# navi0105/LyricAlignment

Measured on AMD Instinct MI355X. Metric: aligned audio-sec/sec (RTF^-1), Whisper-medium 30 s clips, higher is better.
Workload: dtype bf16; 1 GPU; whisper-medium encoder + BiGRU/FC head + CTC forced alignment, batch 32 x 30 s mel per GPU (BASELINE.json configs[1]); clips_per_gpu=32, frames=1500, vocab=21129, labels_per_clip=5..26 (one per sung note), pipeline=2 encoder stream(s) + 1 head stream, head over 4 batches

## Files before the change

lyricalignment_amd/csrc/la_attention.hip:

```cpp
#include <type_traits>

#include "la_common.h"

using la::bf16_t;

namespace {

typedef __attribute__((ext_vector_type(16))) float f32x16;
typedef __attribute__((ext_vector_type(8))) __bf16 bf16x8;
typedef __attribute__((ext_vector_type(8))) _Float16 f16x8;

template <typename T16> struct Half16;
template <> struct Half16<bf16_t> {
    typedef bf16x8 vec8;
    typedef __bf16 elem;
    static constexpr unsigned kOnes = 0x3F803F80u;
    static constexpr float kPLimit = 0x1p30f;
    __device__ static __forceinline__ f32x16 mfma32(vec8 a, vec8 b, f32x16 c) { return __builtin_amdgcn_mfma_f32_32x32x16_bf16(a, b, c, 0, 0, 0); }
};
template <> struct Half16<la::f16_t> {
    typedef f16x8 vec8;
    typedef _Float16 elem;
    static constexpr unsigned kOnes = 0x3C003C00u;
    static constexpr float kPLimit = 0x1p13f;
    __device__ static __forceinline__ f32x16 mfma32(vec8 a, vec8 b, f32x16 c) { return __builtin_amdgcn_mfma_f32_32x32x16_f16(a, b, c, 0, 0, 0); }
};
typedef __attribute__((ext_vector_type(4))) short s16x4;

constexpr int QT = 128;
constexpr int KT = 64;
constexpr float kLog2e = 1.4426950408889634f;

struct AttnParams {
    const void *q, *k, *v;
    int64_t ld_q, ld_kv;
    void *out;
    int64_t ld_out;
    int q_len, kv_len, n_head, causal;
    int64_t q_bs, kv_bs, out_bs;
    int batch;
    float defer_thr;
    float *lse = nullptr;
    float score_scale = 1.4426950408889634f;
};

struct BlockCoord { int qt, head, clip; };
__device__ __forceinline__ BlockCoord block_coord(int nq, int n_head, int batch) {
    const int L = blockIdx.x, pairs = n_head * batch;
    int pair, qt;
    if ((pairs & 7) == 0) {
        const int x = L & 7, idx = L >> 3;
        pair = x + 8 * (idx / nq);
        qt = idx % nq;
    } else {
        pair = L / nq;
        qt = L % nq;
    }
    return BlockCoord{qt, pair % n_head, pair / n_head};
}

__device__ __forceinline__ int acc_row(int reg, int h) { return (reg & 3) + 8 * (reg >> 2) + 4 * h; }

__device__ __forceinline__ void glds16(const void *g, void *l) {
    la::glds16(g, l);
}

__device__ __forceinline__ int kswz(int r) { return (r >> 1) & 7; }
__device__ __forceinline__ int vswz(int r) { return ((r >> 1) & 1) << 2; }

struct KvOff { unsigned k[2], v[2]; };
template <int PER>
__device__ __forceinline__ KvOff kv_offsets_bf16(int64_t ld, int key0, int T, int wave, int lane) {
    KvOff o;
    const int r8 = lane >> 3, ps = lane & 7;
#pragma unroll
    for (int i = 0; i < PER; ++i) {
        const int r = (wave * PER + i) * 8 + r8;
        int rr = key0 + r < T ? r : T - 1 - key0;
        o.k[i] = (unsigned)(rr * ld * 2) + ((ps ^ kswz(r)) << 4);
        o.v[i] = (unsigned)(rr * ld * 2) + ((ps ^ vswz(r)) << 4);
    }
    return o;
}
template <int PER>
__device__ __forceinline__ void stage_kv_bf16(const bf16_t *kbase, const bf16_t *vbase, int64_t ld, int key0, const KvOff &o,
                                              unsigned kl, unsigned vl, int wave) {
    const bf16_t *ks = kbase + (int64_t)key0 * ld, *vs = vbase + (int64_t)key0 * ld;
#pragma unroll
    for (int i = 0; i < PER; ++i) {
        la::glds16_so(o.k[i], ks, kl + (wave * PER + i) * 1024);
        la::glds16_so(o.v[i], vs, vl + (wave * PER + i) * 1024);
    }
}

template <typename T16, int NW = 4, bool MSUM = false, int KO = 0, bool OPT = false, int PRIO = 0, bool FOLD = false>
__global__ __launch_bounds__(64 * NW, FOLD ? 4 : 2) void attention_bf16_kernel(AttnParams p) {
    static_assert(!(OPT && MSUM), "the optimistic form tests the vector-pipe row sums");
    static_assert(!FOLD || OPT, "the log2-domain form is a variant of the optimistic one");
    constexpr int QT = 32 * NW, PER = 8 / NW;
    typedef Half16<T16> HT;
    typedef typename HT::vec8 vec8;
    __shared__ __attribute__((aligned(16))) unsigned char lds[2 * 2 * KT * 128];
    const int T = p.kv_len;
    const BlockCoord bc = block_coord((p.q_len + QT - 1) / QT, p.n_head, p.batch);
    const int qt = bc.qt, head = bc.head, clip = bc.clip;
    const int tid = threadIdx.x, lane = tid & 63;
    const int wave = __builtin_amdgcn_readfirstlane(tid >> 6);
    const int i32 = lane & 31, h = lane >> 5;
    const bf16_t *base = reinterpret_cast<const bf16_t *>(p.q) + (int64_t)clip * p.q_bs * p.ld_q + head * 64;
    const bf16_t *kbase = reinterpret_cast<const bf16_t *>(p.k) + (int64_t)clip * p.kv_bs * p.ld_kv + head * 64;
    const bf16_t *vbase = reinterpret_cast<const bf16_t *>(p.v) + (int64_t)clip * p.kv_bs * p.ld_kv + head * 64;

    int qrow = qt * QT + wave * 32 + i32;
    const bool q_valid = qrow < p.q_len;
    qrow = q_valid ? qrow : p.q_len - 1;
    uint4 qf[4];
#pragma unroll
    for (int c = 0; c < 4; ++c) qf[c] = *reinterpret_cast<const uint4 *>(base + (int64_t)qrow * p.ld_q + 16 * c + 8 * h);

    f32x16 o[2];
#pragma unroll
    for (int b = 0; b < 2; ++b)
#pragma unroll
        for (int r = 0; r < 16; ++r) o[b][r] = 0.f;
    float m_run = FOLD ? 0.f : -INFINITY, l_part = 0.f;
    int plain = FOLD ? 1 : 0;
    const float kScale = FOLD ? 1.0f : p.score_scale;
    f32x16 osum;
#pragma unroll
    for (int r = 0; r < 16; ++r) osum[r] = 0.f;
    const uint4 ones4 = uint4{HT::kOnes, HT::kOnes, HT::kOnes, HT::kOnes};

    int nkv = (T + KT - 1) / KT;
    const int nkv_all = nkv;
    if (p.causal) nkv = min(nkv, (min(p.q_len, (qt + 1) * QT) - 1) / KT + 1);
    const unsigned lds0 = __builtin_amdgcn_readfirstlane(la::lds_addr_u32(lds));
    const KvOff off_full = kv_offsets_bf16<PER>(p.ld_kv, 0, KT, wave, lane);
    const KvOff off_last = kv_offsets_bf16<PER>(p.ld_kv, (nkv_all - 1) * KT, T, wave, lane);
    stage_kv_bf16<PER>(kbase, vbase, p.ld_kv, 0, nkv_all == 1 ? off_last : off_full, lds0, lds0 + KT * 128, wave);
    asm volatile("s_waitcnt vmcnt(0)" ::: "memory");
#pragma unroll
    for (int c = 0; c < 4; ++c) {
        typedef unsigned u32x4 __attribute__((ext_vector_type(4)));
        u32x4 t = __builtin_bit_cast(u32x4, qf[c]);
        asm volatile("" : "+v"(t));
        qf[c] = __builtin_bit_cast(uint4, t);
    }
    __syncthreads();

    const int g = lane >> 4, q4 = (lane & 15) >> 2, pp = lane & 3;

    auto tile = [&](int t, auto curc) __attribute__((always_inline)) {
        constexpr int cur = decltype(curc)::value;
        const unsigned char *kl = lds + cur * (2 * KT * 128);
        const unsigned char *vl = kl + KT * 128;
        if (t + 1 < nkv && !(KO & 8)) {
            const unsigned nk = lds0 + (cur ^ 1) * (2 * KT * 128);
            stage_kv_bf16<PER>(kbase, vbase, p.ld_kv, (t + 1) * KT, t + 2 == nkv_all ? off_last : off_full, nk, nk + KT * 128, wave);
        }
        f32x16 s[2];
        typedef std::integral_constant<int, 0> Sub0;
        typedef std::integral_constant<int, 1> Sub1;
        typedef std::integral_constant<int, 2> SubBoth;
        auto scores = [&](auto serialc, auto whichc) {
            constexpr bool serial = decltype(serialc)::value;
            constexpr int lo = decltype(whichc)::value == 2 ? 0 : decltype(whichc)::value;
            constexpr int hi = decltype(whichc)::value == 2 ? 2 : lo + 1;
            uint4 kf[2][4];
#pragma unroll
            for (int sub = lo; sub < hi; ++sub)
#pragma unroll
                for (int r = 0; r < 16; ++r) s[sub][r] = 0.f;
            if constexpr (!serial) {
#pragma unroll
                for (int c = 0; c < 4; ++c)
#pragma unroll
                    for (int sub = lo; sub < hi; ++sub) {
                        const int row = sub * 32 + i32;
                        if constexpr (KO & 4) kf[sub][c] = qf[(c + sub) & 3];
                        else kf[sub][c] = *reinterpret_cast<const uint4 *>(kl + row * 128 + (((2 * c + h) ^ kswz(row)) << 4));
                    }
            }
#pragma unroll
            for (int c = 0; c < 4; ++c) {
                if constexpr (serial) {
#pragma unroll
                    for (int sub = lo; sub < hi; ++sub) {
                        const int row = sub * 32 + i32;
                        kf[sub][c] = *reinterpret_cast<const uint4 *>(kl + row * 128 + (((2 * c + h) ^ kswz(row)) << 4));
                    }
                }
#pragma unroll
                for (int sub = lo; sub < hi; ++sub)
                    if constexpr (KO & 16) s[sub][c] += __builtin_bit_cast(float, kf[sub][c].x) + __builtin_bit_cast(float, kf[sub][c].w);
                    else s[sub] = HT::mfma32(__builtin_bit_cast(vec8, kf[sub][c]), __builtin_bit_cast(vec8, qf[c]), s[sub]);
                if constexpr (serial) __builtin_amdgcn_sched_barrier(0);
            }
            if ((t + 1) * KT > T || p.causal) {
                const int kmax = p.causal ? min(T - 1, qrow) : T - 1;
#pragma unroll
                for (int sub = lo; sub < hi; ++sub)
#pragma unroll
                    for (int r = 0; r < 16; ++r)
                        if (t * KT + sub * 32 + acc_row(r, h) > kmax) s[sub][r] = -INFINITY;
            }
        };
        typedef float f32x2 __attribute__((ext_vector_type(2)));
        auto exponentials = [&](float m, auto whichc) -> float {
            constexpr int lo = decltype(whichc)::value == 2 ? 0 : decltype(whichc)::value;
            constexpr int hi = decltype(whichc)::value == 2 ? 2 : lo + 1;
            float ps0 = 0.f, ps1 = 0.f;
            auto body = [&](auto subtract_m) {
#pragma unroll
                for (int sub = lo; sub < hi; ++sub)
#pragma unroll
                    for (int r = 0; r < 16; r += 2) {
                        float a0, a1;
                        if constexpr (FOLD) {
                            a0 = s[sub][r]; a1 = s[sub][r + 1];
                            if constexpr (decltype(subtract_m)::value) { a0 -= m; a1 -= m; }
                        } else { a0 = fmaf(s[sub][r], kScale, -m); a1 = fmaf(s[sub][r + 1], kScale, -m); }
                        const float p0 = (KO & 1) ? a0 : __builtin_amdgcn_exp2f(a0), p1 = (KO & 1) ? a1 : __builtin_amdgcn_exp2f(a1);
                        s[sub][r] = p0;
                        s[sub][r + 1] = p1;
                        if constexpr (!MSUM) { ps0 += p0; ps1 += p1; }
                    }
            };
            if (FOLD && plain) body(std::false_type{});
            else body(std::true_type{});
            return ps0 + ps1;
        };
        auto tile_max = [&](auto whichc) -> float {
            constexpr int lo = decltype(whichc)::value == 2 ? 0 : decltype(whichc)::value;
            constexpr int hi = decltype(whichc)::value == 2 ? 2 : lo + 1;
            float mx = -INFINITY;
#pragma unroll
            for (int sub = lo; sub < hi; ++sub)
#pragma unroll
                for (int r = 0; r < 16; ++r) mx = fmaxf(mx, s[sub][r]);
            return fmaxf(mx, __shfl_xor(mx, 32)) * kScale;
        };
        auto rescale = [&](float alpha) {
#pragma unroll
            for (int b = 0; b < 2; ++b)
#pragma unroll
                for (int r = 0; r < 16; ++r) o[b][r] *= alpha;
            if constexpr (MSUM) {
#pragma unroll
                for (int r = 0; r < 16; ++r) osum[r] *= alpha;
            }
        };
        auto pv_sub = [&](auto subc) {
            constexpr int sub = decltype(subc)::value;
#pragma unroll
            for (int ks = 0; ks < 2; ++ks) {
                vec8 pf;
#pragma unroll
                for (int j = 0; j < 8; ++j) pf[j] = (typename HT::elem)s[sub][8 * ks + j];
                if constexpr (MSUM) osum = HT::mfma32(__builtin_bit_cast(vec8, ones4), pf, osum);
#pragma unroll
                for (int b = 0; b < 2; ++b) {
                    const int key0 = sub * 32 + 16 * ks + 4 * (g >> 1);
                    const int slot = b * 4 + 2 * (g & 1) + (pp >> 1);
                    const int r0 = key0 + q4, r1 = key0 + 8 + q4;
                    typedef __attribute__((ext_vector_type(8))) short s16x8;
                    s16x8 vf;
                    if constexpr (KO & 2) vf = __builtin_bit_cast(s16x8, qf[(2 * sub + ks + b) & 3]);
                    else {
                        const s16x4 v0 = __builtin_amdgcn_ds_read_tr16_b64_v4i16(
                            (__attribute__((address_space(3))) s16x4 *)(vl + r0 * 128 + ((slot ^ vswz(r0)) << 4) + (pp & 1) * 8));
                        const s16x4 v1 = __builtin_amdgcn_ds_read_tr16_b64_v4i16(
                            (__attribute__((address_space(3))) s16x4 *)(vl + r1 * 128 + ((slot ^ vswz(r1)) << 4) + (pp & 1) * 8));
                        vf = __builtin_shufflevector(v0, v1, 0, 1, 2, 3, 4, 5, 6, 7);
                    }
                    if constexpr (KO & 16) o[b][2 * sub + ks] += (float)vf[0] + (float)vf[7] + (float)pf[0] + (float)pf[7];
                    else o[b] = HT::mfma32(__builtin_bit_cast(vec8, vf), pf, o[b]);
                }
            }
        };
        auto redo = [&](auto whichc) -> float {
            scores(std::true_type{}, whichc);
            const float m_new = fmaxf(m_run, tile_max(whichc));
            const float alpha = __builtin_amdgcn_exp2f(m_run - m_new);
            m_run = m_new;
            plain = 0;
            rescale(alpha);
            l_part *= alpha;
            return exponentials(m_new, whichc);
        };
        if constexpr (PRIO == 1 || PRIO == 2) __builtin_amdgcn_s_setprio(3);
        scores(std::false_type{}, SubBoth{});
        if constexpr (PRIO == 1 || PRIO == 2) __builtin_amdgcn_s_setprio(0);
        if constexpr (PRIO == 3) __builtin_amdgcn_s_setprio(3);
        if constexpr (OPT) {
            float ps0 = exponentials(m_run, Sub0{});
            if (__builtin_expect(__builtin_amdgcn_ballot_w64(!(ps0 <= HT::kPLimit)) != 0, 0)) ps0 = redo(Sub0{});
            l_part += ps0;
            float ps1 = exponentials(m_run, Sub1{});
            pv_sub(Sub0{});
            if (__builtin_expect(__builtin_amdgcn_ballot_w64(!(ps1 <= HT::kPLimit)) != 0, 0)) ps1 = redo(Sub1{});
            l_part += ps1;
            if constexpr (PRIO == 3) __builtin_amdgcn_s_setprio(0);
            if constexpr (PRIO == 2) __builtin_amdgcn_s_setprio(3);
            pv_sub(Sub1{});
            if constexpr (PRIO == 2) __builtin_amdgcn_s_setprio(0);
        } else {
            const float mx2 = tile_max(SubBoth{});
            float m_new = m_run, alpha = 1.0f;
            if (__builtin_amdgcn_ballot_w64(mx2 > m_run + p.defer_thr) != 0) {
                m_new = fmaxf(m_run, mx2);
                alpha = __builtin_amdgcn_exp2f(m_run - m_new);
            }
            m_run = m_new;
            const float ps = exponentials(m_new, SubBoth{});
            if constexpr (!MSUM) l_part = l_part * alpha + ps;
            if (__builtin_amdgcn_ballot_w64(alpha != 1.0f) != 0) rescale(alpha);
            pv_sub(Sub0{});
            pv_sub(Sub1{});
        }
        asm volatile("s_waitcnt vmcnt(0)" ::: "memory");
        if constexpr (!(KO & 32)) __syncthreads();
    };
    auto sweep = [&]() __attribute__((always_inline)) {
        for (int t = 0; t < nkv; t += 2) {
            tile(t, std::integral_constant<int, 0>{});
            if (t + 1 < nkv) tile(t + 1, std::integral_constant<int, 1>{});
        }
    };
    sweep();
    if constexpr (FOLD) {
        const float l0 = l_part + __shfl_xor(l_part, 32);
        if (__builtin_amdgcn_readfirstlane(__syncthreads_or(q_valid && !(l0 >= 0x1p-100f && l0 <= 0x1p100f)))) {
#pragma unroll
            for (int b = 0; b < 2; ++b)
#pragma unroll
                for (int r = 0; r < 16; ++r) o[b][r] = 0.f;
            m_run = -INFINITY; l_part = 0.f; plain = 0;
            stage_kv_bf16<PER>(kbase, vbase, p.ld_kv, 0, nkv_all == 1 ? off_last : off_full, lds0, lds0 + KT * 128, wave);
            asm volatile("s_waitcnt vmcnt(0)" ::: "memory");
            __syncthreads();
            sweep();
        }
    }

    const float l = MSUM ? osum[0] : l_part + __shfl_xor(l_part, 32);
    const float inv = 1.0f / l;
    if (q_valid) {
        bf16_t *orow = reinterpret_cast<bf16_t *>(p.out) + ((int64_t)clip * p.out_bs + qrow) * p.ld_out + head * 64;
#pragma unroll
        for (int b = 0; b < 2; ++b)
#pragma unroll
            for (int r4 = 0; r4 < 4; ++r4) {
                *reinterpret_cast<ushort4 *>(orow + 32 * b + 8 * r4 + 4 * h) =
                    la::Pack4<T16>::run(o[b][4 * r4 + 0] * inv, o[b][4 * r4 + 1] * inv, o[b][4 * r4 + 2] * inv, o[b][4 * r4 + 3] * inv);
            }
    }
}

__device__ __forceinline__ void stage_kv_f32(const float *kbase, const float *vbase, int64_t ld, int key0, int T,
                                             unsigned char *kl, unsigned char *vl, int wave, int lane) {
    const int r4 = lane >> 4, ps = lane & 15;
#pragma unroll
    for (int i = 0; i < 4; ++i) {
        const int piece = wave * 4 + i;
        const int r = piece * 4 + r4;
        int key = key0 + r;
        key = key < T ? key : T - 1;
        const int ls = ps ^ (r & 15);
        glds16(kbase + (int64_t)key * ld + (ls << 2), kl + piece * 1024);
        glds16(vbase + (int64_t)key * ld + (ls << 2), vl + piece * 1024);
    }
}

__global__ __launch_bounds__(256, 2) void attention_f32_kernel(AttnParams p) {
    extern __shared__ __attribute__((aligned(16))) unsigned char lds[];
    const int T = p.kv_len;
    const BlockCoord bc = block_coord((p.q_len + QT - 1) / QT, p.n_head, p.batch);
    const int qt = bc.qt, head = bc.head, clip = bc.clip;
    const int tid = threadIdx.x, lane = tid & 63, wave = tid >> 6;
    const int i32 = lane & 31, h = lane >> 5;
    const float *base = reinterpret_cast<const float *>(p.q) + (int64_t)clip * p.q_bs * p.ld_q + head * 64;
    const float *kbase = reinterpret_cast<const float *>(p.k) + (int64_t)clip * p.kv_bs * p.ld_kv + head * 64;
    const float *vbase = reinterpret_cast<const float *>(p.v) + (int64_t)clip * p.kv_bs * p.ld_kv + head * 64;

    int qrow = qt * QT + wave * 32 + i32;
    const bool q_valid = qrow < p.q_len;
    qrow = q_valid ? qrow : p.q_len - 1;
    float4 qf[8];
#pragma unroll
    for (int c = 0; c < 8; ++c) qf[c] = *reinterpret_cast<const float4 *>(base + (int64_t)qrow * p.ld_q + 8 * c + 4 * h);

    f32x16 o[2];
#pragma unroll
    for (int b = 0; b < 2; ++b)
#pragma unroll
        for (int r = 0; r < 16; ++r) o[b][r] = 0.f;
    float m_run = -INFINITY, l_part = 0.f;

    constexpr int TILE = KT * 256;
    int nkv = (T + KT - 1) / KT;
    if (p.causal) nkv = min(nkv, (min(p.q_len, (qt + 1) * QT) - 1) / KT + 1);
    stage_kv_f32(kbase, vbase, p.ld_kv, 0, T, lds, lds + TILE, wave, lane);
    asm volatile("s_waitcnt vmcnt(0)" ::: "memory");
    __syncthreads();

    int cur = 0;
// ... 33 lines not shown
#pragma unroll
            for (int r = 0; r < 16; ++r) mx = fmaxf(mx, s[sub][r]);
        mx = fmaxf(mx, __shfl_xor(mx, 32));
        const float m_new = fmaxf(m_run, mx * kLog2e);
        const float alpha = exp2f(m_run - m_new);
        m_run = m_new;
        float psum = 0.f;
#pragma unroll
        for (int sub = 0; sub < 2; ++sub)
#pragma unroll
            for (int r = 0; r < 16; ++r) {
                const float pv = exp2f(fmaf(s[sub][r], kLog2e, -m_new));
                s[sub][r] = pv;
                psum += pv;
            }
        l_part = l_part * alpha + psum;
#pragma unroll
        for (int b = 0; b < 2; ++b)
#pragma unroll
            for (int r = 0; r < 16; ++r) o[b][r] *= alpha;
#pragma unroll
        for (int sub = 0; sub < 2; ++sub)
#pragma unroll
            for (int r = 0; r < 16; ++r) {
                const int key = sub * 32 + acc_row(r, h);
#pragma unroll
                for (int b = 0; b < 2; ++b) {
                    const int col = 32 * b + i32;
                    const float vv = *reinterpret_cast<const float *>(vl + key * 256 + ((((col >> 2) ^ (key & 15)) << 4) | ((col & 3) << 2)));
                    o[b] = __builtin_amdgcn_mfma_f32_32x32x2f32(vv, s[sub][r], o[b], 0, 0, 0);
                }
            }
        asm volatile("s_waitcnt vmcnt(0)" ::: "memory");
        __syncthreads();
        cur ^= 1;
    }

    const float l = l_part + __shfl_xor(l_part, 32);
    const float inv = 1.0f / l;
    if (p.lse && q_valid && h == 0)
        p.lse[((int64_t)clip * p.n_head + head) * p.q_len + qrow] = fmaf(m_run, 0.6931471805599453f, __logf(l));
    if (q_valid) {
        float *orow = reinterpret_cast<float *>(p.out) + ((int64_t)clip * p.out_bs + qrow) * p.ld_out + head * 64;
#pragma unroll
        for (int b = 0; b < 2; ++b)
#pragma unroll
            for (int r4 = 0; r4 < 4; ++r4)
                *reinterpret_cast<float4 *>(orow + 32 * b + 8 * r4 + 4 * h) =
                    make_float4(o[b][4 * r4 + 0] * inv, o[b][4 * r4 + 1] * inv, o[b][4 * r4 + 2] * inv, o[b][4 * r4 + 3] * inv);
    }
}

}

static int attention_launch(int dtype_arg, AttnParams p, int batch, hipStream_t stream) {
    const int dtype = dtype_arg & 0xff;
    const bool qlog2 = dtype_arg & LA_Q_LOG2;
    if (qlog2 && dtype != LA_BF16 && dtype != LA_F16) {
        la::set_error("attention: LA_Q_LOG2 goes with the 16-bit kernels");
        return LA_EINVAL;
    }
    p.score_scale = qlog2 ? 1.0f : kLog2e;
    p.batch = batch;
    const char *thr_env = la::dev_env("LA_ATTN_THR");
    p.defer_thr = thr_env ? (float)atof(thr_env) : 8.0f;
    const dim3 grid(la::cdiv(p.q_len, QT) * p.n_head * batch), block(256);
    if (dtype == LA_BF16 || dtype == LA_F16) {
        la::TimerScope ts("attention_bf16", stream);
        const int nw_opt = la::opts().attn_nw;
        const int nw = nw_opt ? nw_opt : (p.q_len >= 1024 ? 8 : 4);
        const dim3 grid8(la::cdiv(p.q_len, 256) * p.n_head * batch), block8(512);
        const bool wide = nw == 8 && p.q_len >= 256;
#ifdef LA_EXPERIMENTS
        const char *opt_env = getenv("LA_ATTN_OPT"), *fold_env = getenv("LA_ATTN_FOLD");
        const bool no_opt = opt_env && atoi(opt_env) == 0, no_fold = fold_env && atoi(fold_env) == 0;
        if (wide && no_opt) {
            if (dtype == LA_F16) hipLaunchKernelGGL((attention_bf16_kernel<la::f16_t, 8>), grid8, block8, 0, stream, p);
            else hipLaunchKernelGGL((attention_bf16_kernel<bf16_t, 8>), grid8, block8, 0, stream, p);
        } else if (wide && dtype == LA_BF16 && qlog2 && no_fold) {
            hipLaunchKernelGGL((attention_bf16_kernel<bf16_t, 8, false, 0, true>), grid8, block8, 0, stream, p);
        } else if (!wide && getenv("LA_ATTN_MSUM")) {
            if (dtype == LA_F16) hipLaunchKernelGGL((attention_bf16_kernel<la::f16_t, 4, true>), grid, block, 0, stream, p);
            else hipLaunchKernelGGL((attention_bf16_kernel<bf16_t, 4, true>), grid, block, 0, stream, p);
        } else if (!wide && no_opt) {
            if (dtype == LA_F16) hipLaunchKernelGGL((attention_bf16_kernel<la::f16_t, 4>), grid, block, 0, stream, p);
            else hipLaunchKernelGGL((attention_bf16_kernel<bf16_t, 4>), grid, block, 0, stream, p);
        } else if (!wide && dtype == LA_BF16 && qlog2 && no_fold) {
            hipLaunchKernelGGL((attention_bf16_kernel<bf16_t, 4, false, 0, true>), grid, block, 0, stream, p);
        } else
#endif
#ifdef LA_ATTN_KNOCKOUT
        if (const char *ko = getenv("LA_ATTN_KO"); ko && !wide) {
            switch (atoi(ko)) {
#define LA_KO_CASE(n) case n: hipLaunchKernelGGL((attention_bf16_kernel<bf16_t, 4, false, n>), grid, block, 0, stream, p); break;
                LA_KO_CASE(1) LA_KO_CASE(2) LA_KO_CASE(4) LA_KO_CASE(6) LA_KO_CASE(8) LA_KO_CASE(14) LA_KO_CASE(16) LA_KO_CASE(17)
                LA_KO_CASE(7) LA_KO_CASE(15) LA_KO_CASE(30)
#undef LA_KO_CASE
#define LA_KO_OPT(n, ko) case n: { const char *pad = getenv("LA_ATTN_LDSPAD"); \
        hipLaunchKernelGGL((attention_bf16_kernel<bf16_t, 4, false, ko, true>), grid, block, pad ? atoi(pad) : 0, stream, p); } break;
                LA_KO_OPT(132, 32) LA_KO_OPT(140, 40) LA_KO_OPT(100, 0) LA_KO_OPT(101, 1) LA_KO_OPT(106, 6) LA_KO_OPT(108, 8) LA_KO_OPT(114, 14) LA_KO_OPT(116, 16) LA_KO_OPT(130, 30)
#undef LA_KO_OPT
#define LA_KO_PRIO(n, pr) case n: hipLaunchKernelGGL((attention_bf16_kernel<bf16_t, 4, false, 0, true, pr>), grid, block, 0, stream, p); break;
                LA_KO_PRIO(201, 1) LA_KO_PRIO(202, 2) LA_KO_PRIO(203, 3)
#undef LA_KO_PRIO
                default: hipLaunchKernelGGL((attention_bf16_kernel<bf16_t, 4>), grid, block, 0, stream, p);
            }
        } else
#endif
        if (wide) {
            if (dtype == LA_F16) hipLaunchKernelGGL((attention_bf16_kernel<la::f16_t, 8, false, 0, true>), grid8, block8, 0, stream, p);
            else if (qlog2) hipLaunchKernelGGL((attention_bf16_kernel<bf16_t, 8, false, 0, true, 0, true>), grid8, block8, 0, stream, p);
            else hipLaunchKernelGGL((attention_bf16_kernel<bf16_t, 8, false, 0, true>), grid8, block8, 0, stream, p);
        } else if (dtype == LA_F16) hipLaunchKernelGGL((attention_bf16_kernel<la::f16_t, 4, false, 0, true>), grid, block, 0, stream, p);
        else if (qlog2) hipLaunchKernelGGL((attention_bf16_kernel<bf16_t, 4, false, 0, true, 0, true>), grid, block, 0, stream, p);
        else hipLaunchKernelGGL((attention_bf16_kernel<bf16_t, 4, false, 0, true>), grid, block, 0, stream, p);
    } else {
        static la::DeviceOnce attr_once;
        if (attr_once.pending()) {
            LA_HIP(hipFuncSetAttribute(reinterpret_cast<const void *>(attention_f32_kernel),
                                       hipFuncAttributeMaxDynamicSharedMemorySize, 4 * KT * 256));
            attr_once.mark();
        }
        la::TimerScope ts("attention_f32", stream);
        hipLaunchKernelGGL(attention_f32_kernel, grid, block, 4 * KT * 256, stream, p);
    }
    LA_LAUNCH_CHECK();
    return LA_OK;
}

extern "C" int la_attention(int32_t dtype_arg, const void *qkv, int64_t ld_qkv, void *out, int64_t ld_out, int32_t batch,
                            int32_t frames, int32_t n_head, void *stream_) {
    hipStream_t stream = (hipStream_t)stream_;
    if (batch == 0 || frames == 0) return LA_OK;
    LA_CHECK_ARG(qkv && out && batch > 0 && frames > 0 && n_head > 0, "attention: bad arguments");
    const int dtype = dtype_arg & 0xff;
    LA_CHECK_ARG((dtype_arg & ~(0xff | LA_Q_LOG2)) == 0 && (dtype == LA_F32 || dtype == LA_BF16 || dtype == LA_F16), "attention: bad dtype");
    const int es = dtype == LA_F32 ? 4 : 2;
    LA_CHECK_ARG(ld_qkv >= 3 * n_head * 64 && ld_out >= n_head * 64, "attention: leading dimensions too small");
    LA_CHECK_ARG((ld_qkv * es) % 16 == 0 && (ld_out * es) % 16 == 0 && (uintptr_t)qkv % 16 == 0 && (uintptr_t)out % 16 == 0,
                 "attention: rows must be 16-byte aligned");
    const char *b = reinterpret_cast<const char *>(qkv);
    const int d = n_head * 64;
    AttnParams p{b, b + (int64_t)d * es, b + (int64_t)2 * d * es, ld_qkv, ld_qkv, out, ld_out, frames, frames, n_head, 0, frames, frames, frames, 0};
    return attention_launch(dtype_arg, p, batch, stream);
}

extern "C" int la_attention_ex(int32_t dtype_arg, const void *q, int64_t ld_q, const void *k, const void *v, int64_t ld_kv,
                               void *out, int64_t ld_out, int32_t batch, int32_t q_len, int32_t kv_len, int32_t n_head,
                               int32_t causal, void *stream_) {
    hipStream_t stream = (hipStream_t)stream_;
    if (batch == 0 || q_len == 0) return LA_OK;
    LA_CHECK_ARG(q && k && v && out && batch > 0 && q_len > 0 && kv_len > 0 && n_head > 0, "attention_ex: bad arguments");
    const int dtype = dtype_arg & 0xff;
    LA_CHECK_ARG((dtype_arg & ~(0xff | LA_Q_LOG2)) == 0 && (dtype == LA_F32 || dtype == LA_BF16 || dtype == LA_F16), "attention_ex: bad dtype");
    LA_CHECK_ARG(!causal || q_len == kv_len, "attention_ex: causal masking is defined for self-attention (q_len == kv_len)");
    const int es = dtype == LA_F32 ? 4 : 2;
    LA_CHECK_ARG(ld_q >= n_head * 64 && ld_kv >= n_head * 64 && ld_out >= n_head * 64, "attention_ex: leading dimensions too small");
    LA_CHECK_ARG((ld_q * es) % 16 == 0 && (ld_kv * es) % 16 == 0 && (ld_out * es) % 16 == 0 && (uintptr_t)q % 16 == 0 &&
                     (uintptr_t)k % 16 == 0 && (uintptr_t)v % 16 == 0 && (uintptr_t)out % 16 == 0,
                 "attention_ex: rows must be 16-byte aligned");
    AttnParams p{q, k, v, ld_q, ld_kv, out, ld_out, q_len, kv_len, n_head, causal ? 1 : 0, q_len, kv_len, q_len, 0};
    return attention_launch(dtype_arg, p, batch, stream);
}

extern "C" int la_attention_lse_f32(const float *q, int64_t ld_q, const float *k, const float *v, int64_t ld_kv, float *out, int64_t ld_out,
                                    int32_t batch, int32_t q_len, int32_t kv_len, int32_t n_head, int32_t causal, float *lse, void *stream_) {
// ... 31 lines not shown
```

lyricalignment_amd/csrc/la_common.h:

```cpp
#pragma once
#include <hip/hip_runtime.h>
#include <stdint.h>
#include <stdio.h>
#include <stdlib.h>
#include <string.h>

#include "../../include/lyricalign.h"

namespace la {

char *err_buf();
void set_error(const char *fmt, ...);

enum { SCRATCH_SPLITK = 0, SCRATCH_COLSUM = 1, SCRATCH_X2 = 2 };
void *stream_scratch(hipStream_t stream, int purpose, size_t bytes);

#define LA_CHECK_ARG(cond, ...)                \
    do {                                       \
        if (!(cond)) {                         \
            la::set_error(__VA_ARGS__);        \
            return LA_EINVAL;                  \
        }                                      \
    } while (0)

#define LA_HIP(expr)                                                                     \
    do {                                                                                 \
        hipError_t _e = (expr);                                                          \
        if (_e != hipSuccess) {                                                          \
            la::set_error("%s:%d %s -> %s", __FILE__, __LINE__, #expr, hipGetErrorString(_e)); \
            return LA_EHIP;                                                              \
        }                                                                                \
    } while (0)

#define LA_LAUNCH_CHECK()                                                               \
    do {                                                                                \
        hipError_t _e = hipGetLastError();                                              \
        if (_e != hipSuccess) {                                                         \
            la::set_error("%s:%d launch -> %s", __FILE__, __LINE__, hipGetErrorString(_e)); \
            return LA_EHIP;                                                             \
        }                                                                               \
    } while (0)

struct Options {
    int gemm_tile = 0, gemm_loop = 0, gemm_splitk = 1, attn_nw = 0, gru_nw = 0, gru_fence = 0, gru_handoff = 0, gru_poll_delay = 0, viterbi_dpp = 1,
        head_clip_cap = 0, ln_fusion = 1, resid_split = 1, x2_inference = 1, gru_timeout_us = 0, gru_fault_step = 0, x2_small = 0;
};
Options &opts();
#ifdef LA_EXPERIMENTS
inline const char *dev_env(const char *name) { return getenv(name); }
#define LA_DEV_BIT(word, bits) ((word) & (bits))
#else
inline const char *dev_env(const char *) { return nullptr; }
#define LA_DEV_BIT(word, bits) false
#endif

struct DeviceOnce {
    unsigned long long done[4] = {0, 0, 0, 0};
    static int current() {
        int d = 0;
        if (hipGetDevice(&d) != hipSuccess) d = 0;
        return d & 255;
    }
    bool pending() const {
        const int d = current();
        return !((__atomic_load_n(&done[d >> 6], __ATOMIC_ACQUIRE) >> (d & 63)) & 1ull);
    }
    void mark() {
        const int d = current();
        __atomic_fetch_or(&done[d >> 6], 1ull << (d & 63), __ATOMIC_RELEASE);
    }
};

struct TimerScope {
    bool active;
    hipStream_t stream;
    TimerScope(const char *family, hipStream_t s, double work = 0.0);
    ~TimerScope();
};

int gemm_run(int dtype, int M, int N, int K, int batch, const void *A, int64_t lda, int64_t strideA, const void *W,
             int64_t strideW, void *C, int64_t ldc, int64_t strideC, const float *bias, int64_t strideBias,
             const float *residual, int64_t ldr, int64_t strideR, int epilogue, hipStream_t stream);

inline int64_t round_up(int64_t x, int64_t m) { return (x + m - 1) / m * m; }
inline int cdiv(int64_t a, int64_t b) { return (int)((a + b - 1) / b); }

typedef unsigned short bf16_t;

__device__ __forceinline__ float bf16_to_f32(bf16_t v) { return __uint_as_float(((unsigned)v) << 16); }

__device__ __forceinline__ bf16_t f32_to_bf16(float f) {
    __bf16 b = (__bf16)f;
    return __builtin_bit_cast(unsigned short, b);
}

typedef _Float16 f16_t;

// ... 102 lines not shown
    p = __builtin_elementwise_fma(p, t, f32x2{1.477083683e+00f, 1.477083683e+00f});
    p = __builtin_elementwise_fma(p, t, f32x2{-1.828017831e+00f, -1.828017831e+00f});
    const f32x2 y2 = __builtin_elementwise_fma(x * f32x2{-0.72134752044f, -0.72134752044f}, x, p);
    const f32x2 e = {__builtin_amdgcn_exp2f(y2.x), __builtin_amdgcn_exp2f(y2.y)};
    const f32x2 u = __builtin_elementwise_fma(-ax, t * e, ax);
    return (x + u) * f32x2{0.5f, 0.5f};
}

__device__ __forceinline__ float gelu_sig(float x) {
    const float xc = __builtin_amdgcn_fmed3f(x, -8.0f, 8.0f);
    const float s = xc * xc;
    float p = fmaf(1.0148166172e-03f, s, -1.0677913190e-01f);
    p = fmaf(p, s, -2.3011175945e+00f);
    const float e = __builtin_amdgcn_exp2f(p * xc);
    return x * __builtin_amdgcn_rcpf(1.0f + e);
}

__device__ __forceinline__ f32x2 gelu_sig2(f32x2 x) {
    const f32x2 xc = {__builtin_amdgcn_fmed3f(x.x, -8.0f, 8.0f), __builtin_amdgcn_fmed3f(x.y, -8.0f, 8.0f)};
    const f32x2 s = xc * xc;
    f32x2 p = __builtin_elementwise_fma(f32x2{1.0148166172e-03f, 1.0148166172e-03f}, s, f32x2{-1.0677913190e-01f, -1.0677913190e-01f});
    p = __builtin_elementwise_fma(p, s, f32x2{-2.3011175945e+00f, -2.3011175945e+00f});
    const f32x2 z = p * xc;
    const f32x2 e = {__builtin_amdgcn_exp2f(z.x), __builtin_amdgcn_exp2f(z.y)};
    const f32x2 d = e + f32x2{1.0f, 1.0f};
    const f32x2 r = {__builtin_amdgcn_rcpf(d.x), __builtin_amdgcn_rcpf(d.y)};
    return x * r;
}

__device__ __forceinline__ float mish(float x) {
    float sp = x > 20.0f ? x : log1pf(expf(x));
    return x * tanhf(sp);
}

__device__ __forceinline__ void glds16(const void *gsrc, const void *lds_base) {
    const unsigned dst = __builtin_amdgcn_readfirstlane((unsigned)(uintptr_t)(const __attribute__((address_space(3))) void *)lds_base);
    unsigned keep;
    asm volatile("s_mov_b32 %0, m0\n\ts_mov_b32 m0, %2\n\ts_nop 0\n\tglobal_load_lds_dwordx4 %1, off\n\ts_mov_b32 m0, %0"
                 : "=&s"(keep)
                 : "v"(gsrc), "s"(dst)
                 : "memory");
}

__device__ __forceinline__ void glds16_so(unsigned voff, const void *sbase, unsigned m0_dst) {
    asm volatile("s_mov_b32 m0, %2\n\ts_nop 0\n\tglobal_load_lds_dwordx4 %0, %1"
                 :
                 : "v"(voff), "s"(sbase), "s"(m0_dst)
                 : "memory");
}
__device__ __forceinline__ unsigned lds_addr_u32(const void *p) {
    return (unsigned)(uintptr_t)(const __attribute__((address_space(3))) void *)p;
}

__device__ __forceinline__ float sigmoidf_(float x) { return 1.0f / (1.0f + expf(-x)); }

}
```

lyricalignment_amd/csrc/la_runtime.cpp:

```cpp
#include <stdarg.h>
#include <stdlib.h>

#include <mutex>
#include <string>
#include <vector>

#include "la_common.h"

namespace la {

char *err_buf() {
    static thread_local char buf[512] = {0};
    return buf;
}

void set_error(const char *fmt, ...) {
    va_list ap;
    va_start(ap, fmt);
    vsnprintf(err_buf(), 512, fmt, ap);
    va_end(ap);
}

void *stream_scratch(hipStream_t stream, int purpose, size_t bytes) {
    struct Slot { int dev; hipStream_t stream; int purpose; void *ptr; size_t bytes; };
    static std::mutex mu;
    static std::vector<Slot> slots;
    int dev = 0;
    if (hipGetDevice(&dev) != hipSuccess) return nullptr;
    std::lock_guard<std::mutex> lock(mu);
    for (Slot &sl : slots)
        if (sl.dev == dev && sl.stream == stream && sl.purpose == purpose) {
            if (sl.bytes >= bytes) return sl.ptr;
            if (hipStreamSynchronize(stream) != hipSuccess) return nullptr;
            (void)hipFree(sl.ptr);
            sl.ptr = nullptr; sl.bytes = 0;
            if (hipMalloc(&sl.ptr, bytes) != hipSuccess) return nullptr;
            sl.bytes = bytes;
            return sl.ptr;
        }
    Slot sl{dev, stream, purpose, nullptr, bytes < ((size_t)1 << 20) ? ((size_t)1 << 20) : bytes};
    if (hipMalloc(&sl.ptr, sl.bytes) != hipSuccess) return nullptr;
    slots.push_back(sl);
    return sl.ptr;
}

namespace {
struct OptionDesc { const char *name, *env; int Options::*field; bool env_inverts; };
const OptionDesc kOptions[] = {
    {"gemm_tile", "LA_GEMM_TILE", &Options::gemm_tile, false},       {"gemm_loop", "LA_PP_DBG", &Options::gemm_loop, false},
    {"gemm_splitk", "LA_GEMM_NO_SPLITK", &Options::gemm_splitk, true}, {"attn_nw", "LA_ATTN_NW", &Options::attn_nw, false},
    {"gru_nw", "LA_GRU_NW", &Options::gru_nw, false},                 {"gru_fence", "LA_GRU_FENCE", &Options::gru_fence, false},
    {"gru_handoff", "LA_GRU_HANDOFF", &Options::gru_handoff, false}, {"gru_poll_delay", "LA_GRU_POLL_DELAY", &Options::gru_poll_delay, false},
    {"viterbi_dpp", "LA_VITERBI_NO_DPP", &Options::viterbi_dpp, true}, {"head_clip_cap", "LA_HEAD_CLIP_CAP", &Options::head_clip_cap, false},
    {"ln_fusion", "LA_LN_FUSION", &Options::ln_fusion, false},       {"resid_split", "LA_RESID_SPLIT", &Options::resid_split, false},
    {"x2_inference", "LA_X2_INFERENCE", &Options::x2_inference, false}, {"x2_small", "LA_X2_SMALL", &Options::x2_small, false},
    {"gru_timeout_us", "LA_GRU_TIMEOUT_US", &Options::gru_timeout_us, false}, {"gru_fault_step", "LA_GRU_FAULT_STEP", &Options::gru_fault_step, false},
};
}

Options &opts() {
    static Options o = [] {
        Options v;
        for (const OptionDesc &d : kOptions) {
            const char *e = getenv(d.env);
            if (!e) continue;
            v.*(d.field) = d.env_inverts ? 0 : atoi(e);
        }
        return v;
    }();
    return o;
}

namespace {
struct TimerState {
    std::mutex mu;
    bool enabled = false;
    std::string family;
    std::vector<std::pair<hipEvent_t, hipEvent_t>> pairs;
    std::vector<std::pair<hipEvent_t, hipEvent_t>> pool;
    int period = 1;
    int64_t seen = 0;
    double work = 0.0;
};
TimerState &ts() {
    static TimerState s;
    return s;
}
}

TimerScope::TimerScope(const char *family, hipStream_t s, double work) : active(false), stream(s) {
    TimerState &t = ts();
    if (!t.enabled) return;
    std::lock_guard<std::mutex> lk(t.mu);
    if (!t.enabled || t.family != family) return;
    if (t.seen++ % t.period != 0) return;
    std::pair<hipEvent_t, hipEvent_t> pr;
    if (!t.pool.empty()) {
        pr = t.pool.back();
        t.pool.pop_back();
    } else {
        if (hipEventCreate(&pr.first) != hipSuccess) return;
        if (hipEventCreate(&pr.second) != hipSuccess) { (void)hipEventDestroy(pr.first); return; }
    }
    (void)hipEventRecord(pr.first, stream);
    t.pairs.push_back(pr);
    t.work += work;
    active = true;
}

// ... 115 lines not shown
```

Baseline: 23620 audio-sec/sec.

## Add lean attention loop variants with dead-wave skipping and tail-tile specialization

```diff
diff --git a/lyricalignment_amd/csrc/la_attention.hip b/lyricalignment_amd/csrc/la_attention.hip
--- a/lyricalignment_amd/csrc/la_attention.hip
+++ b/lyricalignment_amd/csrc/la_attention.hip
@@ -69,34 +69,36 @@
 __device__ __forceinline__ int vswz(int r) { return ((r >> 1) & 1) << 2; }
 
 struct KvOff { unsigned k[2], v[2]; };
-template <int PER>
-__device__ __forceinline__ KvOff kv_offsets_bf16(int64_t ld, int key0, int T, int wave, int lane) {
+template <int PER, int PS = 1>
+__device__ __forceinline__ KvOff kv_offsets_bf16(int64_t ld, int key0, int T, int piece0, int lane) {
     KvOff o;
     const int r8 = lane >> 3, ps = lane & 7;
 #pragma unroll
     for (int i = 0; i < PER; ++i) {
-        const int r = (wave * PER + i) * 8 + r8;
+        const int r = (piece0 + i * PS) * 8 + r8;
         int rr = key0 + r < T ? r : T - 1 - key0;
         o.k[i] = (unsigned)(rr * ld * 2) + ((ps ^ kswz(r)) << 4);
         o.v[i] = (unsigned)(rr * ld * 2) + ((ps ^ vswz(r)) << 4);
     }
     return o;
 }
-template <int PER>
+template <int PER, int PS = 1>
 __device__ __forceinline__ void stage_kv_bf16(const bf16_t *kbase, const bf16_t *vbase, int64_t ld, int key0, const KvOff &o,
-                                              unsigned kl, unsigned vl, int wave) {
+                                              unsigned kl, unsigned vl, int piece0) {
     const bf16_t *ks = kbase + (int64_t)key0 * ld, *vs = vbase + (int64_t)key0 * ld;
 #pragma unroll
     for (int i = 0; i < PER; ++i) {
-        la::glds16_so(o.k[i], ks, kl + (wave * PER + i) * 1024);
-        la::glds16_so(o.v[i], vs, vl + (wave * PER + i) * 1024);
-    }
-}
-
-template <typename T16, int NW = 4, bool MSUM = false, int KO = 0, bool OPT = false, int PRIO = 0, bool FOLD = false>
+        la::glds16_so(o.k[i], ks, kl + (piece0 + i * PS) * 1024);
+        la::glds16_so(o.v[i], vs, vl + (piece0 + i * PS) * 1024);
+    }
+}
+
+template <typename T16, int NW = 4, bool MSUM = false, int KO = 0, bool OPT = false, int PRIO = 0, bool FOLD = false, int LEAN = 0>
 __global__ __launch_bounds__(64 * NW, FOLD ? 4 : 2) void attention_bf16_kernel(AttnParams p) {
     static_assert(!(OPT && MSUM), "the optimistic form tests the vector-pipe row sums");
     static_assert(!FOLD || OPT, "the log2-domain form is a variant of the optimistic one");
+    static_assert(!LEAN || (FOLD && KO == 0 && PRIO == 0), "the lean loop is a variant of the shipped log2-domain form");
+    constexpr bool PLACED = LEAN == 3;
     constexpr int QT = 32 * NW, PER = 8 / NW;
     typedef Half16<T16> HT;
     typedef typename HT::vec8 vec8;
@@ -112,8 +114,10 @@
     const bf16_t *vbase = reinterpret_cast<const bf16_t *>(p.v) + (int64_t)clip * p.kv_bs * p.ld_kv + head * 64;
 
     int qrow = qt * QT + wave * 32 + i32;
-    const bool q_valid = qrow < p.q_len;
+    bool q_valid = qrow < p.q_len;
     qrow = q_valid ? qrow : p.q_len - 1;
+    int h_out = h;
+    const bool dead = LEAN && qt * QT + wave * 32 >= p.q_len;
     uint4 qf[4];
 #pragma unroll
     for (int c = 0; c < 4; ++c) qf[c] = *reinterpret_cast<const uint4 *>(base + (int64_t)qrow * p.ld_q + 16 * c + 8 * h);
@@ -135,9 +139,28 @@
     const int nkv_all = nkv;
     if (p.causal) nkv = min(nkv, (min(p.q_len, (qt + 1) * QT) - 1) / KT + 1);
     const unsigned lds0 = __builtin_amdgcn_readfirstlane(la::lds_addr_u32(lds));
-    const KvOff off_full = kv_offsets_bf16<PER>(p.ld_kv, 0, KT, wave, lane);
-    const KvOff off_last = kv_offsets_bf16<PER>(p.ld_kv, (nkv_all - 1) * KT, T, wave, lane);
-    stage_kv_bf16<PER>(kbase, vbase, p.ld_kv, 0, nkv_all == 1 ? off_last : off_full, lds0, lds0 + KT * 128, wave);
+    constexpr int PS = PLACED && PER == 2 ? 2 : 1;
+    const int piece0 = PS == 2 ? (wave & 1) + 4 * (wave >> 1) : wave * PER;
+    const unsigned placed_off_k = (unsigned)((piece0 * 8 + (lane >> 3)) * p.ld_kv * 2) + (((lane & 7) ^ kswz(piece0 * 8 + (lane >> 3))) << 4);
+    const unsigned placed_off_v = (unsigned)((piece0 * 8 + (lane >> 3)) * p.ld_kv * 2) + (((lane & 7) ^ vswz(piece0 * 8 + (lane >> 3))) << 4);
+    KvOff off_full, off_last;
+    auto make_offsets = [&](int lane_o) {
+        off_full = kv_offsets_bf16<PER, PS>(p.ld_kv, 0, KT, piece0, lane_o);
+        off_last = kv_offsets_bf16<PER, PS>(p.ld_kv, (nkv_all - 1) * KT, T, piece0, lane_o);
+    };
+    auto stage_placed = [&](int t1, unsigned nk) {
+        const bf16_t *ks = kbase + (int64_t)t1 * KT * p.ld_kv, *vs = vbase + (int64_t)t1 * KT * p.ld_kv;
+#pragma unroll
+        for (int i = 0; i < PER; ++i) {
+            la::glds16_so(placed_off_k, ks + (int64_t)(16 * i) * p.ld_kv, nk + (piece0 + 2 * i) * 1024);
+            la::glds16_so(placed_off_v, vs + (int64_t)(16 * i) * p.ld_kv, nk + KT * 128 + (piece0 + 2 * i) * 1024);
+        }
+    };
+    if constexpr (PLACED) stage_placed(0, lds0);
+    else {
+        make_offsets(lane);
+        stage_kv_bf16<PER, PS>(kbase, vbase, p.ld_kv, 0, nkv_all == 1 ? off_last : off_full, lds0, lds0 + KT * 128, piece0);
+    }
     asm volatile("s_waitcnt vmcnt(0)" ::: "memory");
 #pragma unroll
     for (int c = 0; c < 4; ++c) {
@@ -150,13 +173,19 @@
 
     const int g = lane >> 4, q4 = (lane & 15) >> 2, pp = lane & 3;
 
-    auto tile = [&](int t, auto curc) __attribute__((always_inline)) {
-        constexpr int cur = decltype(curc)::value;
+    auto tile = [&](int t, auto curc, auto modec) __attribute__((always_inline)) -> int {
+        constexpr int MODE = decltype(modec)::value;
+        int lane_t = lane;
+        if constexpr (PLACED && MODE != 3) asm volatile("" : "+v"(lane_t));
+        const int i32 = lane_t & 31, h = lane_t >> 5, g = lane_t >> 4, q4 = (lane_t & 15) >> 2, pp = lane_t & 3;
+        const int cur = decltype(curc)::value == 2 ? (t & 1) : decltype(curc)::value;
         const unsigned char *kl = lds + cur * (2 * KT * 128);
         const unsigned char *vl = kl + KT * 128;
-        if (t + 1 < nkv && !(KO & 8)) {
+        if constexpr (MODE == 3) {
+            if (t + 1 < nkv) stage_placed(t + 1, lds0 + (cur ^ 1) * (2 * KT * 128));
+        } else if (t + 1 < nkv && !(KO & 8) && (MODE == 0 || MODE == 4)) {
             const unsigned nk = lds0 + (cur ^ 1) * (2 * KT * 128);
-            stage_kv_bf16<PER>(kbase, vbase, p.ld_kv, (t + 1) * KT, t + 2 == nkv_all ? off_last : off_full, nk, nk + KT * 128, wave);
+            stage_kv_bf16<PER, PS>(kbase, vbase, p.ld_kv, (t + 1) * KT, t + 2 == nkv_all ? off_last : off_full, nk, nk + KT * 128, piece0);
         }
         f32x16 s[2];
         typedef std::integral_constant<int, 0> Sub0;
@@ -215,6 +244,18 @@
                 for (int sub = lo; sub < hi; ++sub)
 #pragma unroll
                     for (int r = 0; r < 16; r += 2) {
+                        if constexpr (LEAN >= 2) {
+                            if (r & 2) continue;
+                            float a[4];
+#pragma unroll
+                            for (int j = 0; j < 4; ++j) {
+                                a[j] = s[sub][r + j];
+                                if constexpr (decltype(subtract_m)::value) a[j] -= m;
+                                s[sub][r + j] = __builtin_amdgcn_exp2f(a[j]);
+                            }
+                            la::add4_f32_single(ps0, ps1, s[sub][r], s[sub][r + 1], s[sub][r + 2], s[sub][r + 3]);
+                            continue;
+                        }
                         float a0, a1;
                         if constexpr (FOLD) {
                             a0 = s[sub][r]; a1 = s[sub][r + 1];
@@ -288,6 +329,87 @@
             l_part *= alpha;
             return exponentials(m_new, whichc);
         };
+        if constexpr (MODE == 3) {
+            typedef __attribute__((ext_vector_type(8))) short s16x8;
+            auto kread = [&](int sub, int c) -> uint4 {
+                const int row = sub * 32 + i32;
+                return *reinterpret_cast<const uint4 *>(kl + row * 128 + (((2 * c + h) ^ kswz(row)) << 4));
+            };
+            auto vread = [&](int sub, int i) -> s16x8 {
+                const int ks = i >> 1, b = i & 1;
+                const int key0 = sub * 32 + 16 * ks + 4 * (g >> 1);
+                const int slot = b * 4 + 2 * (g & 1) + (pp >> 1);
+                const int r0 = key0 + q4, r1 = key0 + 8 + q4;
+                const s16x4 v0 = __builtin_amdgcn_ds_read_tr16_b64_v4i16(
+                    (__attribute__((address_space(3))) s16x4 *)(vl + r0 * 128 + ((slot ^ vswz(r0)) << 4) + (pp & 1) * 8));
+                const s16x4 v1 = __builtin_amdgcn_ds_read_tr16_b64_v4i16(
+                    (__attribute__((address_space(3))) s16x4 *)(vl + r1 * 128 + ((slot ^ vswz(r1)) << 4) + (pp & 1) * 8));
+                return __builtin_shufflevector(v0, v1, 0, 1, 2, 3, 4, 5, 6, 7);
+            };
+            auto softmax4 = [&](int sub, int c, float &a0, float &a1, vec8 *pf) {
+#pragma unroll
+                for (int j = 0; j < 4; ++j) s[sub][4 * c + j] = __builtin_amdgcn_exp2f(s[sub][4 * c + j]);
+                la::add4_f32_single(a0, a1, s[sub][4 * c], s[sub][4 * c + 1], s[sub][4 * c + 2], s[sub][4 * c + 3]);
+#pragma unroll
+                for (int j = 0; j < 4; ++j) pf[c >> 1][4 * (c & 1) + j] = (typename HT::elem)s[sub][4 * c + j];
+            };
+            constexpr bool DEEP = NW == 8;
+            uint4 k0[4], k1[4];
+            s16x8 vf[4];
+            vec8 pf0[2], pf1[2];
+#pragma unroll
+            for (int c = 0; c < 4; ++c) k0[c] = kread(0, c);
+#pragma unroll
+            for (int sub = 0; sub < 2; ++sub)
+#pragma unroll
+                for (int r = 0; r < 16; ++r) s[sub][r] = 0.f;
+            __builtin_amdgcn_sched_barrier(0);
+#pragma unroll
+            for (int c = 0; c < 4; ++c) {
+                s[0] = HT::mfma32(__builtin_bit_cast(vec8, k0[c]), __builtin_bit_cast(vec8, qf[c]), s[0]);
+                if (DEEP || c < 2) k1[c] = kread(1, c);
+                __builtin_amdgcn_sched_barrier(0);
+            }
+            float a0 = 0.f, a1 = 0.f;
+#pragma unroll
+            for (int c = 0; c < 4; ++c) {
+                s[1] = HT::mfma32(__builtin_bit_cast(vec8, k1[c]), __builtin_bit_cast(vec8, qf[c]), s[1]);
+                if (!DEEP && c < 2) k1[c + 2] = kread(1, c + 2);
+                if (c >= 2) { vf[2 * c - 4] = vread(0, 2 * c - 4); vf[2 * c - 3] = vread(0, 2 * c - 3); }
+                __builtin_amdgcn_sched_barrier(0);
+                softmax4(0, c, a0, a1, pf0);
+                __builtin_amdgcn_sched_barrier(0);
+            }
+            const float ps0 = a0 + a1;
+            if (__builtin_expect(__builtin_amdgcn_ballot_w64(!(ps0 <= HT::kPLimit)) != 0, 0)) return 1;
+            l_part += ps0;
+            a0 = 0.f; a1 = 0.f;
+            s16x8 vg[4];
+#pragma unroll
+            for (int i = 0; i < 4; ++i) {
+                o[i & 1] = HT::mfma32(__builtin_bit_cast(vec8, vf[i]), pf0[i >> 1], o[i & 1]);
+                if constexpr (DEEP) vg[i] = vread(1, i);
+                else if (i >= 2) { vg[2 * i - 4] = vread(1, 2 * i - 4); vg[2 * i - 3] = vread(1, 2 * i - 3); }
+                __builtin_amdgcn_sched_barrier(0);
+                softmax4(1, i, a0, a1, pf1);
+                __builtin_amdgcn_sched_barrier(0);
+            }
+            const float ps1 = a0 + a1;
+            if (__builtin_expect(__builtin_amdgcn_ballot_w64(!(ps1 <= HT::kPLimit)) != 0, 0)) return 2;
+            l_part += ps1;
+#pragma unroll
+            for (int i = 0; i < 4; ++i) o[i & 1] = HT::mfma32(__builtin_bit_cast(vec8, vg[i]), pf1[i >> 1], o[i & 1]);
+        } else if constexpr (MODE == 2) {
+            const float ps1 = redo(Sub1{});
+            l_part += ps1;
+            pv_sub(Sub1{});
+        } else if ((PLACED || MODE == 4) && t + 1 == nkv_all && T - t * KT <= 32) {
+            scores(std::false_type{}, Sub0{});
+            float ps0 = exponentials(m_run, Sub0{});
+            if (__builtin_expect(__builtin_amdgcn_ballot_w64(!(ps0 <= HT::kPLimit)) != 0, 0)) ps0 = redo(Sub0{});
+            l_part += ps0;
+            pv_sub(Sub0{});
+        } else {
         if constexpr (PRIO == 1 || PRIO == 2) __builtin_amdgcn_s_setprio(3);
         scores(std::false_type{}, SubBoth{});
         if constexpr (PRIO == 1 || PRIO == 2) __builtin_amdgcn_s_setprio(0);
@@ -318,16 +440,81 @@
             pv_sub(Sub0{});
             pv_sub(Sub1{});
         }
+        }
         asm volatile("s_waitcnt vmcnt(0)" ::: "memory");
         if constexpr (!(KO & 32)) __syncthreads();
+        return 0;
     };
-    auto sweep = [&]() __attribute__((always_inline)) {
-        for (int t = 0; t < nkv; t += 2) {
-            tile(t, std::integral_constant<int, 0>{});
-            if (t + 1 < nkv) tile(t + 1, std::integral_constant<int, 1>{});
+    typedef std::integral_constant<int, 0> Buf0;
+    typedef std::integral_constant<int, 1> Buf1;
+    typedef std::integral_constant<int, 2> BufOfT;
+    typedef std::integral_constant<int, 0> General;
+    typedef std::integral_constant<int, 3> Placed;
+    auto sweep = [&](int t0) __attribute__((always_inline)) {
+        if constexpr (LEAN == 1 || LEAN == 2) {
+            if (dead) {
+                for (int t = 0; t < nkv; ++t) {
+                    if (t + 1 < nkv) {
+                        const unsigned nk = lds0 + ((t & 1) ^ 1) * (2 * KT * 128);
+                        stage_kv_bf16<PER, PS>(kbase, vbase, p.ld_kv, (t + 1) * KT, t + 2 == nkv_all ? off_last : off_full, nk, nk + KT * 128, piece0);
+                    }
+                    asm volatile("s_waitcnt vmcnt(0)" ::: "memory");
+                    __syncthreads();
+                }
+            } else {
+                for (int t = 0; t + 1 < nkv; t += 2) {
+                    tile(t, Buf0{}, General{});
+                    if (t + 2 < nkv) tile(t + 1, Buf1{}, General{});
+                }
+                tile(nkv - 1, BufOfT{}, std::integral_constant<int, 4>{});
+            }
+        } else if constexpr (PLACED) {
+            int lane_o = lane;
+            asm volatile("" : "+v"(lane_o));
+            make_offsets(lane_o);
+            if (dead) {
+                for (int t = t0; t < nkv; ++t) {
+                    if (t + 1 < nkv) {
+                        const unsigned nk = lds0 + ((t & 1) ^ 1) * (2 * KT * 128);
+                        stage_kv_bf16<PER, PS>(kbase, vbase, p.ld_kv, (t + 1) * KT, t + 2 == nkv_all ? off_last : off_full, nk, nk + KT * 128, piece0);
+                    }
+                    asm volatile("s_waitcnt vmcnt(0)" ::: "memory");
+                    __syncthreads();
+                }
+            } else {
+                for (int t = t0; t < nkv; ++t) tile(t, BufOfT{}, General{});
+            }
+        } else {
+            for (int t = t0; t < nkv; t += 2) {
+                tile(t, Buf0{}, General{});
+                if (t + 1 < nkv) tile(t + 1, Buf1{}, General{});
+            }
         }
     };
-    sweep();
+    int t_done = 0;
+    if constexpr (PLACED) {
+        const int nfast = dead ? 0 : (T % KT ? T / KT - 1 : T / KT);
+        int left = 0;
+        while (t_done + 1 < nfast) {
+            left = tile(t_done, Buf0{}, Placed{});
+            if (left) break;
+            ++t_done;
+            left = tile(t_done, Buf1{}, Placed{});
+            if (left) break;
+            ++t_done;
+        }
+        if (!left && t_done < nfast) {
+            left = tile(t_done, Buf0{}, Placed{});
+            if (!left) ++t_done;
+        }
+        if (left) {
+            if (left == 1) tile(t_done, BufOfT{}, std::integral_constant<int, 1>{});
+            else tile(t_done, BufOfT{}, std::integral_constant<int, 2>{});
+            ++t_done;
+        }
+    }
+    sweep(t_done);
+    {
     if constexpr (FOLD) {
         const float l0 = l_part + __shfl_xor(l_part, 32);
         if (__builtin_amdgcn_readfirstlane(__syncthreads_or(q_valid && !(l0 >= 0x1p-100f && l0 <= 0x1p100f)))) {
@@ -336,13 +523,22 @@
 #pragma unroll
                 for (int r = 0; r < 16; ++r) o[b][r] = 0.f;
             m_run = -INFINITY; l_part = 0.f; plain = 0;
-            stage_kv_bf16<PER>(kbase, vbase, p.ld_kv, 0, nkv_all == 1 ? off_last : off_full, lds0, lds0 + KT * 128, wave);
+            stage_kv_bf16<PER, PS>(kbase, vbase, p.ld_kv, 0, nkv_all == 1 ? off_last : off_full, lds0, lds0 + KT * 128, piece0);
             asm volatile("s_waitcnt vmcnt(0)" ::: "memory");
             __syncthreads();
-            sweep();
-        }
-    }
-
+            sweep(0);
+        }
+    }
+    }
+
+    if constexpr (PLACED) {
+        int lane_e = lane;
+        asm volatile("" : "+v"(lane_e));
+        qrow = qt * QT + wave * 32 + (lane_e & 31);
+        q_valid = qrow < p.q_len;
+        qrow = q_valid ? qrow : p.q_len - 1;
+        h_out = lane_e >> 5;
+    }
     const float l = MSUM ? osum[0] : l_part + __shfl_xor(l_part, 32);
     const float inv = 1.0f / l;
     if (q_valid) {
@@ -351,7 +547,7 @@
         for (int b = 0; b < 2; ++b)
 #pragma unroll
             for (int r4 = 0; r4 < 4; ++r4) {
-                *reinterpret_cast<ushort4 *>(orow + 32 * b + 8 * r4 + 4 * h) =
+                *reinterpret_cast<ushort4 *>(orow + 32 * b + 8 * r4 + 4 * (PLACED ? h_out : h)) =
                     la::Pack4<T16>::run(o[b][4 * r4 + 0] * inv, o[b][4 * r4 + 1] * inv, o[b][4 * r4 + 2] * inv, o[b][4 * r4 + 3] * inv);
             }
     }
@@ -491,6 +687,8 @@
 }
 
 }
+
+constexpr int kLeanDefault = 2;
 
 static int attention_launch(int dtype_arg, AttnParams p, int batch, hipStream_t stream) {
     const int dtype = dtype_arg & 0xff;
@@ -510,6 +708,9 @@
         const int nw = nw_opt ? nw_opt : (p.q_len >= 1024 ? 8 : 4);
         const dim3 grid8(la::cdiv(p.q_len, 256) * p.n_head * batch), block8(512);
         const bool wide = nw == 8 && p.q_len >= 256;
+        const int loop_opt = la::opts().attn_loop;
+        const int lean = !(dtype == LA_BF16 && qlog2 && !p.causal && p.q_len == p.kv_len && p.kv_len >= KT) || loop_opt == 1 ? 0
+                         : loop_opt >= 2 && loop_opt <= 4 ? loop_opt - 1 : kLeanDefault;
 #ifdef LA_EXPERIMENTS
         const char *opt_env = getenv("LA_ATTN_OPT"), *fold_env = getenv("LA_ATTN_FOLD");
         const bool no_opt = opt_env && atoi(opt_env) == 0, no_fold = fold_env && atoi(fold_env) == 0;
@@ -548,9 +749,15 @@
 #endif
         if (wide) {
             if (dtype == LA_F16) hipLaunchKernelGGL((attention_bf16_kernel<la::f16_t, 8, false, 0, true>), grid8, block8, 0, stream, p);
+            else if (lean == 1) hipLaunchKernelGGL((attention_bf16_kernel<bf16_t, 8, false, 0, true, 0, true, 1>), grid8, block8, 0, stream, p);
+            else if (lean == 2) hipLaunchKernelGGL((attention_bf16_kernel<bf16_t, 8, false, 0, true, 0, true, 2>), grid8, block8, 0, stream, p);
+            else if (lean == 3) hipLaunchKernelGGL((attention_bf16_kernel<bf16_t, 8, false, 0, true, 0, true, 3>), grid8, block8, 0, stream, p);
             else if (qlog2) hipLaunchKernelGGL((attention_bf16_kernel<bf16_t, 8, false, 0, true, 0, true>), grid8, block8, 0, stream, p);
             else hipLaunchKernelGGL((attention_bf16_kernel<bf16_t, 8, false, 0, true>), grid8, block8, 0, stream, p);
         } else if (dtype == LA_F16) hipLaunchKernelGGL((attention_bf16_kernel<la::f16_t, 4, false, 0, true>), grid, block, 0, stream, p);
+        else if (lean == 1) hipLaunchKernelGGL((attention_bf16_kernel<bf16_t, 4, false, 0, true, 0, true, 1>), grid, block, 0, stream, p);
+        else if (lean == 2) hipLaunchKernelGGL((attention_bf16_kernel<bf16_t, 4, false, 0, true, 0, true, 2>), grid, block, 0, stream, p);
+        else if (lean == 3) hipLaunchKernelGGL((attention_bf16_kernel<bf16_t, 4, false, 0, true, 0, true, 3>), grid, block, 0, stream, p);
         else if (qlog2) hipLaunchKernelGGL((attention_bf16_kernel<bf16_t, 4, false, 0, true, 0, true>), grid, block, 0, stream, p);
         else hipLaunchKernelGGL((attention_bf16_kernel<bf16_t, 4, false, 0, true>), grid, block, 0, stream, p);
     } else {
diff --git a/lyricalignment_amd/csrc/la_common.h b/lyricalignment_amd/csrc/la_common.h
--- a/lyricalignment_amd/csrc/la_common.h
+++ b/lyricalignment_amd/csrc/la_common.h
@@ -42,7 +42,7 @@
     } while (0)
 
 struct Options {
-    int gemm_tile = 0, gemm_loop = 0, gemm_splitk = 1, attn_nw = 0, gru_nw = 0, gru_fence = 0, gru_handoff = 0, gru_poll_delay = 0, viterbi_dpp = 1,
+    int gemm_tile = 0, gemm_loop = 0, gemm_splitk = 1, attn_nw = 0, attn_loop = 0, gru_nw = 0, gru_fence = 0, gru_handoff = 0, gru_poll_delay = 0, viterbi_dpp = 1,
         head_clip_cap = 0, ln_fusion = 1, resid_split = 1, x2_inference = 1, gru_timeout_us = 0, gru_fault_step = 0, x2_small = 0;
 };
 Options &opts();
@@ -251,6 +251,12 @@
     return (unsigned)(uintptr_t)(const __attribute__((address_space(3))) void *)p;
 }
 
+__device__ __forceinline__ void add4_f32_single(float &acc0, float &acc1, float x0, float x1, float x2, float x3) {
+    asm("s_nop 0\n\tv_add_f32 %0, %0, %2\n\tv_add_f32 %1, %1, %3\n\tv_add_f32 %0, %0, %4\n\tv_add_f32 %1, %1, %5"
+        : "+v"(acc0), "+v"(acc1)
+        : "v"(x0), "v"(x1), "v"(x2), "v"(x3));
+}
+
 __device__ __forceinline__ float sigmoidf_(float x) { return 1.0f / (1.0f + expf(-x)); }
 
 }
diff --git a/lyricalignment_amd/csrc/la_runtime.cpp b/lyricalignment_amd/csrc/la_runtime.cpp
--- a/lyricalignment_amd/csrc/la_runtime.cpp
+++ b/lyricalignment_amd/csrc/la_runtime.cpp
@@ -55,6 +55,7 @@
     {"ln_fusion", "LA_LN_FUSION", &Options::ln_fusion, false},       {"resid_split", "LA_RESID_SPLIT", &Options::resid_split, false},
     {"x2_inference", "LA_X2_INFERENCE", &Options::x2_inference, false}, {"x2_small", "LA_X2_SMALL", &Options::x2_small, false},
     {"gru_timeout_us", "LA_GRU_TIMEOUT_US", &Options::gru_timeout_us, false}, {"gru_fault_step", "LA_GRU_FAULT_STEP", &Options::gru_fault_step, false},
+    {"attn_loop", "LA_ATTN_LOOP", &Options::attn_loop, false},
 };
 }
 
```

Result: no change. 23770 audio-sec/sec (median of 6 runs) (+0.6%).
